# itsdevbear/go-avalanche

Measured on AMD Instinct MI355X. Metric: vote-record updates/sec (node·target·round) at 1/2/4/8 GPU; % HBM roofline, higher is better.
Workload: dtype u32; 1 GPU; C4: 1M nodes x 1000 targets, k=8, Bernoulli(0.8) initial acceptance, honest, sim mode; n_nodes=1000000, n_targets=1000, k=8, parallelism=single GPU

## Files before the change

go-avalanche_amd/csrc/engine.cpp:

```cpp
#include <algorithm>
#include <cstdarg>
#include <cstdio>
#include <cstring>
#include <memory>
#include <string>
#include <utility>
#include <vector>

#include "engine.h"

using namespace aveng;

namespace aveng {

static thread_local std::string g_last_error;

int fail(int code, const char* fmt, ...) {
  char buf[512];
  va_list ap;
  va_start(ap, fmt);
  vsnprintf(buf, sizeof(buf), fmt, ap);
  va_end(ap);
  g_last_error = buf;
  return code;
// ... 41 lines not shown
  p.log_shards = e->log_shards;
  p.n_nodes = (uint32_t)e->N;
  p.n0 = (uint32_t)e->n0;
  p.NL = e->NL;
  p.BL = e->BL;
  p.PS = e->PS;
  p.L = e->L;
  p.Lpad = e->Lpad;
  p.t0 = (uint32_t)e->t0;
  p.round = (uint32_t)e->round;
  p.round_rel = (uint32_t)(e->round - e->log_base);
  p.round_shift = e->round_shift;
  p.peer_mode = e->cfg.peer_mode;
  p.warm_all = e->facts.warm_all ? 1u : 0u;
  p.store_policy = e->store_policy;
  p.bl_magic = e->bl_magic;
  p.bl_sh1 = e->bl_sh1;
  p.bl_sh2 = e->bl_sh2;
  p.kpend = e->kpend;
  p.tn = (uint32_t)(e->t1 - e->t0);
  p.nopipe = e->sweep_nopipe ? 1u : 0u;
  p.tpw = e->wave_runs && e->sweep_blocks ? 1u : 0u;
  p.settled_fast = e->settled_fast ? 1u : 0u;
  p.lean = e->settled_lean && 64 % e->BL == 0 ? 1u : 0u;
  p.bl_log2 = (uint32_t)__builtin_ctz(e->BL);
  p.pub_mode = (uint32_t)e->pub_mode;
  p.readd = e->pub_mode == 2 ? e->readd : nullptr;
  p.died_out = e->pub_mode == 2 ? e->died_out : nullptr;
  p.nopoll = e->any_nopoll ? e->nopoll : nullptr;
  p.dense_min = e->dense_min;
  p.wave_dense = e->wave_dense;
  p.uni_votes = e->uni_votes;
  p.quiet_tiles = e->quiet_tiles;
  return p;
}

int materialize(av_engine* e, bool votes, bool counts) {
  votes = votes && e->facts.v_stale;
  counts = counts && e->facts.k_pend;
  if (!votes && !counts) return AV_OK;
  AV_HIP(avk::launch_materialize(round_params(e, nullptr), votes, counts, e->stream));
  if (votes) e->facts.votes_written_back();
  if (counts) e->facts.counts_written_back();
  return AV_OK;
}
int materialize_votes(av_engine* e) { return materialize(e, true, true); }

int engine_scratch(av_engine* e, size_t bytes, void** out) {
  const hipError_t he = e->fetch_scratch.reserve(bytes);
  AV_CHECK(he == hipSuccess, oom_or_hip(he), "scratch (%zu B): %s", bytes, hipGetErrorString(he));
  *out = e->fetch_scratch;
  return AV_OK;
}

int ref_pick(av_engine* e) {
  if (e->ref_node != -1) return AV_OK;
  e->ref_node = -2;
  const size_t words = std::min<size_t>((e->N + 31) / 32, 1024);
  std::vector<uint32_t> w(words);
  AV_HIP(hipMemcpyAsync(w.data(), e->byz, words * 4, hipMemcpyDeviceToHost, e->stream));
  AV_HIP(hipStreamSynchronize(e->stream));
  for (size_t i = 0; i < words && e->ref_node < 0; ++i)
    if (~w[i]) {
      const int64_t n = (int64_t)i * 32 + __builtin_ctz(~w[i]);
      if (n < e->N) e->ref_node = n;
    }
// ... 378 lines not shown
  e->log_shards = (uint32_t)std::max<uint64_t>(1, std::min<uint64_t>(waves, avk::kLogShards));
  e->log_cap = (uint32_t)std::max<int64_t>((cap + e->log_shards - 1) / e->log_shards, 64);
  AV_TRY(created(e->planes.alloc(plane_words), "alloc planes"));
  e->rflag_off = (pref_words * 4 + 255) / 256 * 256;
  e->uni_off = (e->rflag_off + (size_t)e->N + 255) / 256 * 256 / 4;
  e->pref_alloc_words =
      ((e->uni_off * 4 + (avk::kMaxPeers + 1) * 4 + (2u << 20) - 1) / (2u << 20)) * (2u << 20) / 4;
  for (auto& pref : e->pref) AV_TRY(created(pref.alloc_zeroed(e->pref_alloc_words, s), "alloc pref"));
  AV_TRY(created(e->vstale.alloc_zeroed(e->Lpad / 64, s), "alloc planes"));
  AV_TRY(created(e->kpend.alloc_zeroed(e->Lpad / 64, s), "alloc planes"));
  AV_TRY(created(e->valid.alloc(e->BL), "alloc valid"));
  AV_TRY(created(e->byz.alloc((e->N + 31) / 32), "alloc byz"));
  AV_TRY(created(e->log.alloc((size_t)e->log_cap * e->log_shards), "alloc log"));
  AV_TRY(created(e->log_count.alloc_zeroed(3 * avk::kLogShards * avk::kCtrStride, s), "alloc log"));
  e->mlog_count = e->log_count + avk::kLogShards * avk::kCtrStride;
  e->dlog_count = e->log_count + 2 * avk::kLogShards * avk::kCtrStride;
  const uint32_t dw = avk::dense_words((uint32_t)e->k);
  e->dense_min = avk::dense_min((uint32_t)e->k);
  const uint32_t dense_least = e->k == 8 ? 4u : e->dense_min;
  e->dlog_cap = std::max<uint32_t>(e->log_cap / dense_least, 16);
  AV_TRY(created(e->dlog.alloc((size_t)e->dlog_cap * e->log_shards * dw), "alloc log"));
  AV_TRY(created(e->upd_count.alloc_zeroed(avk::kLogShards, s), "alloc log"));
  e->mlog_cap = e->k == 8 ? std::max<uint32_t>(e->log_cap / 2, 16) : 16u;
  AV_TRY(created(e->mlog.alloc((size_t)e->mlog_cap * e->log_shards * avk::med_rec_words()), "alloc log"));
  e->log_alloc = (size_t)e->log_cap * e->log_shards;
  e->mlog_alloc = (size_t)e->mlog_cap * e->log_shards;
  e->dlog_alloc = (size_t)e->dlog_cap * e->log_shards;
  AV_TRY(created(e->log_overflow.alloc_zeroed(1, s), "alloc log"));
  if (e->capped) AV_TRY(created(e->node_flags.alloc_zeroed(e->NL, s), "alloc node flags"));
  AV_TRY(created(e->applied.alloc_zeroed(avk::kLogShards, s), "alloc counters"));
  AV_TRY(created(e->bytes.alloc_zeroed(2 * avk::kLogShards, s), "alloc counters"));
  AV_TRY(created(e->finalized.alloc_zeroed(avk::kLogShards, s), "alloc counters"));
  AV_TRY(created(e->scratch_count.alloc(1), "alloc counters"));
  AV_TRY(created(e->changed.alloc_zeroed(3 * avk::kLogShards, s), "alloc counters"));
  AV_TRY(created(e->nq.alloc_zeroed(4, s), "alloc counters"));
  e->valid_host.assign(e->BL, 0u);
  for (uint32_t b = 0; b < e->BL; ++b) {
    const int64_t tb = e->t0 + 32ll * b;
    const int64_t r = std::min<int64_t>(e->t1 - tb, 32);
    e->valid_host[b] = r >= 32 ? ~0u : ((1u << r) - 1u);
  }
  AV_TRY(created(hipMemcpyAsync(e->valid, e->valid_host.data(), e->BL * 4, hipMemcpyHostToDevice, s), "upload valid"));
  AV_TRY(created(avk::launch_byz(e->byz, (uint32_t)e->N, c.seed, c.byz_threshold, s), "byz kernel"));
  e->sweep_blocks = default_sweep_blocks(e);
  set_log_layout(e);
  AV_TRY(av_init_records(e, AV_INIT_NONE, 0));
  *out = guard.release();
  return AV_OK;
}

int av_init_records(av_engine* e, int32_t init_mode, uint32_t init_param) {
  AV_ENTER(e);
  AV_CHECK(init_mode >= AV_INIT_NONE && init_mode <= AV_INIT_PAIRS, AV_ERR_INVALID_ARG, "bad init_mode");
  if (e->facts.v_stale) AV_HIP(hipMemsetAsync(e->vstale, 0, (size_t)(e->Lpad / 64) * 4, e->stream));
  if (e->facts.k_pend) AV_HIP(hipMemsetAsync(e->kpend, 0, (size_t)(e->Lpad / 64) * 4, e->stream));
  e->facts.init(init_mode != AV_INIT_NONE);
  avk::InitParams p{};
  p.planes = e->planes;
  p.pref = e->pref[e->cur];
  p.byz = e->byz;
  p.seed = e->cfg.seed;
  p.n_nodes = (uint32_t)e->N;
  p.n0 = (uint32_t)e->n0;
  p.NL = e->NL;
  p.BL = e->BL;
  p.PS = e->PS;
  p.L = e->L;
// ... 149 lines not shown
  return {n, kd, lo, hi, nullptr, nullptr, m};
}

constexpr PlainOption kPlainOptions[] = {
    opt("plane_nt", &av_engine::plane_nt),
    opt("uniform_rows", &av_engine::uni_rows),
    opt("ref_rows", &av_engine::ref_rows),
    opt("virtual_votes", &av_engine::virtual_votes),
    opt("vv_min_bl", &av_engine::vv_min_bl, kReject, 1, (1ll << 31) - 1),
    opt("kernel", &av_engine::kernel, kReject, 1, 2),
    opt("store_policy", &av_engine::store_policy, kReject, 0, 3),
    opt("settled_fast", &av_engine::settled_fast),
    opt("settled_lean", &av_engine::settled_lean),
    opt("wave_runs", &av_engine::wave_runs),
    opt("sweep_nopipe", &av_engine::sweep_nopipe),
    opt("uni_merge", &av_engine::uni_merge, kReject, 1, 16),
    opt("uni_votes", &av_engine::uni_votes),
    opt("quiet_tiles", &av_engine::quiet_tiles),
    opt("net_quiet", &av_engine::net_quiet),
    opt("net_quiet_group", &av_engine::nq_group, kReject, 1, 16),
    opt("net_quiet_front", &av_engine::nq_front),
    opt("wave_dense", &av_engine::wave_dense, kReject, 0, 64),
    opt("tile_draw", &av_engine::tile_draw, kReject, 0, 1),
    opt("materialize_run", &av_engine::mat_run, kReject, 1, 64),
    opt("replay_fuse", &av_engine::replay_fuse, kReject, 0, 4096),
    opt("replay_fast", &av_engine::replay_fast),
    opt("dropin_fast", &av_engine::dropin_fast),
    opt("push_defer", &av_engine::push_defer),
    opt("push_store", &av_engine::push_store, kReject, 0, 2),
    opt("census_blocks", &av_engine::census_blocks, kReject, 0, 65536),
    opt("copy_blocks", &av_engine::copy_blocks, kReject, 0, 4096),
    opt("enc_buckets", &av_engine::enc_buckets, kReject, 1, 1ll << 30),
    opt("count_changed", &av_engine::count_changed),
    opt("round_marker", &av_engine::round_marker),
    opt("warm_pref", &av_engine::warm_pref),
    opt("unsynced_shard", &av_engine::unsynced_shard),
    opt("ablate_gather", &av_engine::ablate_gather),
    opt("ablate_phase", &av_engine::ablate_phase, kClamp, 0, 31),
    opt("ablate_emit", &av_engine::ablate_emit, kClamp, 0, 3),
    opt("ablate_node", &av_engine::ablate_node, kClamp, 0, 7),
};

int opt_range(const char* name, int64_t value, int64_t lo, int64_t hi) {
  AV_CHECK(value >= lo && value <= hi, AV_ERR_INVALID_ARG, "%s must be in [%lld, %lld]", name, (long long)lo,
           (long long)hi);
  return AV_OK;
}

int set_plain(av_engine* e, const PlainOption& o, int64_t value) {
  if (o.kind == kReject) AV_TRY(opt_range(o.name, value, o.lo, o.hi));
  value = o.kind == kBool ? value != 0 : std::max(o.lo, std::min(o.hi, value));
  if (o.b)
    e->*o.b = value != 0;
  else if (o.u)
    e->*o.u = (uint32_t)value;
  else
    e->*o.i = (int)value;
  return AV_OK;
}

int opt_sweep_blocks(av_engine* e, int64_t value) {
  AV_TRY(opt_range("sweep_blocks", value, -2, (1ll << 31) - 1));
  AV_ENTER(e);
  e->sweep_blocks = value < 0 ? default_sweep_blocks(e, value == -2) : (uint32_t)value;
  e->sweep_blocks_explicit = value >= 0;
  return relayout_log_if_empty(e);
// ... 148 lines not shown
```

go-avalanche_amd/csrc/engine.h:

```cpp
#pragma once

#include <hip/hip_runtime.h>
#include <rccl/rccl.h>

#include <algorithm>
#include <cstdint>
#include <cstdlib>
#include <thread>
#include <utility>
#include <vector>

#pragma GCC visibility push(default)
#include "../../include/avhip.h"
#pragma GCC visibility pop
#include "engine_mem.h"
#include "kernels.h"
#include "round_plan.h"

namespace aveng {
int fail(int code, const char* fmt, ...) __attribute__((format(printf, 2, 3)));
inline int oom_or_hip(hipError_t he) { return he == hipErrorOutOfMemory ? AV_ERR_OOM : AV_ERR_HIP; }
}

#define AV_HIP(call)                                                                                           \
// ... 120 lines not shown
  bool pref_uncached = false;
  bool peer_fine = true;
  size_t pref_alloc_words = 0;
  uint32_t barrier_seq = 0;
  uint32_t barrier_timeout_ms = 30000;
  std::vector<void*> peer_opened;
  avk::PeerPtrs peer_arrive{};
  avmem::DevBuf<uint32_t*> push_tbl;
  uint64_t barrier_ticks = 0;
  bool solo_barrier = false;
  bool solo_used = false;
  PeerGroup* group = nullptr;
  bool peer_mask = true;
  bool push_defer = true;
  uint32_t push_store = 1;
  uint32_t tile_draw = 0;
  uint32_t mat_run = 1;
  uint32_t census_blocks = 0;
  bool masked = false;
  uint32_t segs = 1;
  avmem::DevBuf<uint8_t> need_mine;
  avmem::DevBuf<uint8_t> needmask;
  avmem::DevBuf<uint8_t> stale;
  uint32_t* needin = nullptr;
  avmem::DevBuf<uint32_t> needin_own;
  avk::PeerPtrs peer_needin{};
  int64_t need_ready = -1;
  int64_t need_pushed = -1;
  avmem::Stream need_stream;
  avmem::Event need_free, need_drawn;
  int64_t need_drawn_w = -1;
  avmem::DevBuf<unsigned long long> changed;
  bool count_changed = false;
  int64_t rflag_clear_round = 0;

  uint32_t dense_min = 0;
  uint32_t wave_dense = 0;
  uint32_t uni_votes = 1;
  uint32_t quiet_tiles = 1;
  uint32_t net_quiet = 1;
  uint32_t nq_group = 16;
  uint32_t nq_front = 1;
  avmem::DevBuf<uint32_t> nq;
  int32_t pub_mode = 0;
  avmem::DevBuf<uint32_t> readd;
  avmem::DevBuf<uint32_t> died_out;
  std::vector<uint32_t> nopoll_host;
  avmem::DevBuf<uint32_t> nopoll;
  bool any_nopoll = false;
  std::vector<int64_t> proc_round;
  avmem::DevBuf<void> fetch_scratch;
  avmem::DevBuf<unsigned long long> digest;
  avmem::PinnedBuf<void> dropin_host;
  avmem::PinnedBuf<void> stage[2];
  avmem::Event stage_ev[2];
  bool dropin_fast = true;
  avmem::DevBuf<uint32_t> enc_err;
  avmem::DevBuf<uint64_t> enc_tot;
  uint32_t enc_buckets = 1u << 26;
  uint32_t copy_blocks = 0;
  static constexpr int kSlots = 3;
  avmem::Stream copy_stream;
  avmem::DevBuf<uint8_t> cdev[kSlots];
  avmem::PinnedBuf<uint8_t> chost[kSlots];
  avmem::Event cev[kSlots];
  av_compact_header chdr[kSlots] = {};
// ... 70 lines not shown
```

go-avalanche_amd/csrc/engine_records.cpp:

```cpp
#include <cstring>

#include "engine.h"

using namespace aveng;

namespace {

int peer_local_write_check(const av_engine* e) {
  AV_CHECK(e->peer_world <= 1, AV_ERR_UNSUPPORTED,
           "record writes outside a round are not supported on a peer-push node-sharded engine");
  return AV_OK;
}

int sum_shards(av_engine* e, const unsigned long long* dev, int64_t* out) {
  std::vector<unsigned long long> c(avk::kLogShards);
  AV_HIP(hipMemcpyAsync(c.data(), dev, avk::kLogShards * 8, hipMemcpyDeviceToHost, e->stream));
  AV_HIP(hipStreamSynchronize(e->stream));
  unsigned long long t = 0;
  for (auto v : c) t += v;
  *out = (int64_t)t;
  return AV_OK;
}

}
// ... 409 lines not shown
  if (out->target_classes) {
    const int64_t counted = (int64_t)h[tn * 4 + 256];
    for (size_t t = 0; t < tn; ++t) {
      int64_t* row = out->target_classes + t * AV_CENSUS_CLASSES;
      row[AV_CENSUS_LIVE_REJECTED] = (int64_t)h[t * 3];
      row[AV_CENSUS_LIVE_ACCEPTED] = (int64_t)h[t * 3 + 1];
      row[AV_CENSUS_ABSENT_ACCEPTED] = (int64_t)h[t * 3 + 2];
      row[AV_CENSUS_ABSENT_REJECTED] = counted - row[0] - row[1] - row[3];
    }
  }
  if (out->target_count_sum)
    for (size_t t = 0; t < tn; ++t) out->target_count_sum[t] = (int64_t)h[tn * 3 + t];
  if (out->count_hist)
    for (size_t i = 0; i < 256; ++i) out->count_hist[i] = (int64_t)h[tn * 4 + i];
  return AV_OK;
}

int av_alg_bytes(av_engine* e, int64_t* out) {
  AV_TRY(counter_query(e, out));
  return sum_shards(e, e->bytes, out);
}

int av_alg_bytes_reread(av_engine* e, int64_t* out) {
  AV_TRY(counter_query(e, out));
  return sum_shards(e, e->bytes + avk::kLogShards, out);
}

int av_changed_words(av_engine* e, int64_t* words, int64_t* segments) {
  AV_TRY(counter_query(e, words));
  AV_TRY(sum_shards(e, e->changed, words));
  return segments ? sum_shards(e, e->changed + avk::kLogShards, segments) : AV_OK;
}

int av_net_quiet_rounds(av_engine* e, int64_t* out) {
  AV_TRY(counter_query(e, out));
  uint32_t v = 0;
  AV_HIP(hipMemcpyAsync(&v, e->nq + 2, 4, hipMemcpyDeviceToHost, e->stream));
  AV_HIP(hipStreamSynchronize(e->stream));
  *out = (int64_t)v;
  return AV_OK;
}

int av_read_pref(av_engine* e, int64_t n0, int64_t n1, int64_t t0, int64_t t1, uint8_t* out) {
  AV_ENTER(e);
  AV_PEER_SYNC_CHECK(e);
  AV_CHECK(out && n0 >= 0 && n0 <= n1 && n1 <= e->N && t0 >= e->t0 && t0 <= t1 && t1 <= e->t1,
           AV_ERR_INVALID_ARG, "bad range");
  const size_t rows = (size_t)(n1 - n0);
  std::vector<uint32_t> w(rows * e->BL);
  if (rows) AV_TRY(av_read_pref_words(e, n0, n1, w.data()));
  const int64_t W = t1 - t0;
  for (size_t r = 0; r < rows; ++r)
    for (int64_t t = t0; t < t1; ++t) {
      const int64_t tl = t - e->t0;
      out[r * W + (t - t0)] = (uint8_t)((w[r * e->BL + (tl >> 5)] >> (tl & 31)) & 1u);
    }
  return AV_OK;
}

int av_read_pref_words(av_engine* e, int64_t n0, int64_t n1, uint32_t* out) {
  AV_ENTER(e);
  AV_PEER_SYNC_CHECK(e);
  AV_CHECK(out && n0 >= 0 && n0 <= n1 && n1 <= e->N, AV_ERR_INVALID_ARG, "bad range");
  const size_t words = (size_t)(n1 - n0) * e->BL;
  if (!words) return AV_OK;
  AV_HIP(hipMemcpy2DAsync(out, (size_t)e->BL * 4, e->pref[e->cur] + (size_t)n0 * e->PS, (size_t)e->PS * 4,
// ... 26 lines not shown
```

go-avalanche_amd/csrc/kernels.h:

```cpp
#pragma once

#include <hip/hip_runtime.h>
#include <stdint.h>

namespace avk {

constexpr int kPlanes = 25;
constexpr int kPV = 0, kPC = 8, kPA = 16, kPK = 17;
constexpr uint32_t kLogShards = 1024;
constexpr uint32_t kCtrStride = 32;
constexpr uint32_t kMaxPoll = 4096;
constexpr int kMaxK = 16;
constexpr int kMaxPeers = 15;

__host__ __device__ constexpr size_t replay_groups(int k) { return (size_t)((k + 1) / 2); }
__host__ __device__ inline size_t replay_words(uint32_t Lpad, int k) { return replay_groups(k) * 4u * Lpad; }
__host__ __device__ inline size_t replay_idx(uint32_t g, int k, int j, int c) {
  return (((size_t)(g >> 6) * replay_groups(k) + (size_t)(j >> 1)) * 64u + (g & 63u)) * 4u + (size_t)((j & 1) * 2 + c);
}

__host__ __device__ constexpr uint32_t pref_stride(uint32_t BL) {
  return BL > 32u ? (BL + 31u) / 32u * 32u : (BL <= 1u ? 1u : 1u << (32 - __builtin_clz(BL - 1u)));
}

// ... 77 lines not shown
  uint32_t ps_shift;
  const uint8_t* rflag_in;
  uint8_t* rflag_out;
  uint32_t rflag_off;

  uint32_t* uni_out;
  const uint32_t* uni_in;
  const uint32_t* uni_prev;
  uint32_t uni_world, uni_rank, uni_off;
  uint32_t uni_merge;
  uint32_t uni_post;

  uint32_t fresh;
  uint32_t tn;
  uint32_t hivirt;
  uint32_t tpw;
  uint32_t settled_fast;
  uint32_t lean;
  uint32_t bl_log2;
  uint32_t nopipe;
  uint32_t pub_mode;
  uint32_t* readd;
  uint32_t* died_out;
  const uint32_t* nopoll;
  uint32_t dense_min;
  uint32_t uni_votes;
  uint32_t quiet_tiles;
  uint32_t* nq_out;
  const uint32_t* nq_in;
  uint32_t* nq_rounds;
  uint32_t nq_group;
  uint32_t nq_front;
  uint32_t wave_dense;
};
constexpr uint32_t kPendAllLive = 0x80000000u;
constexpr uint32_t kHiVirt = 0x40000000u;
__host__ __device__ inline uint32_t real_mask(uint32_t tn, uint32_t b) {
  const uint32_t rem = tn > b * 32u ? tn - b * 32u : 0u;
  return rem >= 32u ? ~0u : ((1u << rem) - 1u);
}
constexpr uint32_t kVStale = 1u, kVUniform = 2u, kVMask = 3u, kCAll = 4u;

inline void bl_divider(uint32_t d, uint32_t& magic, uint32_t& sh1, uint32_t& sh2) {
  uint32_t l = 0;
  while ((1ull << l) < d) ++l;
  magic = (uint32_t)((((1ull << l) - d) << 32) / d + 1);
  sh1 = l < 1 ? l : 1;
  sh2 = l > 1 ? l - 1 : 0;
}

__host__ __device__ constexpr uint32_t dense_words(uint32_t k) { return (k + 5u) / 2u; }
__host__ __device__ constexpr uint32_t dense_min(uint32_t k) { return dense_words(k); }

constexpr uint32_t kMedS4Died = 1u << 8;
__host__ __device__ constexpr uint32_t med_rec_words() { return 4u; }

__host__ __device__ inline uint64_t pack_update(uint32_t round_rel, uint32_t node, uint32_t slot,
                                                uint32_t target, uint32_t status, uint32_t round_shift) {
  return ((uint64_t)round_rel << round_shift) | ((uint64_t)node << 28) | ((uint64_t)slot << 24) |
         ((uint64_t)target << 2) | (uint64_t)status;
}

hipError_t launch_round(const RoundParams& p, int k, bool replay, bool capped, hipStream_t s);
hipError_t launch_replay_node(const RoundParams& p, int k, hipStream_t s);
enum class SweepMode : int;
hipError_t launch_round_sweep(const RoundParams& p, int k, SweepMode mode, uint32_t blocks, hipStream_t s,
// ... 145 lines not shown
```

go-avalanche_amd/csrc/round_sweep.hip:

```cpp
#include <hip/hip_runtime.h>

#include <algorithm>

#include "kernels.h"
#include "round_common.h"
#include "round_plan.h"
#include "round_slots.h"

#ifndef AVK_ABLATE_PHASE
#define AVK_ABLATE_PHASE 0
#endif
#ifndef AVK_PUB_PRELOAD
#define AVK_PUB_PRELOAD 0
#endif

namespace avk {
namespace {

constexpr bool kAblatePhase = AVK_ABLATE_PHASE != 0;

struct SweepAcc {
  uint32_t applied = 0, died = 0, lane_bytes = 0;
  uint32_t reread = 0;
  uint32_t emitted_bytes = 0, updates = 0;
// ... 223 lines not shown
        if (in.stale == kVStale && (uflags & kUniPrev)) {
          const uint32_t rp = at_byte(p.pref_prev, p.ref_node * rb + bo);
          in.v0 = u32x4{rp, rp, rp, rp};
          in.v1 = u32x4{rp, rp, rp, 0u};
        } else if (in.stale == kVStale) {
          uint32_t pp[K];
          pick_parked(p, wd->sdp, wd->badp, base, x.node, p.round - 1u, rb, pp);
#pragma unroll
          for (int i = 0; i < 4; ++i) in.v0[i] = nog ? pp[7 - i] * 0x9E3779B9u : at_byte(p.pref_prev, pp[7 - i] + bo);
#pragma unroll
          for (int i = 0; i < 3; ++i) in.v1[i] = nog ? pp[3 - i] * 0x9E3779B9u : at_byte(p.pref_prev, pp[3 - i] + bo);
          in.v1[3] = 0u;
        }
        pick_parked(p, wd->sdc, wd->badc, base, x.node, p.round, rb, rows);
        drawn = have_rows = true;
        if (nog) {
#pragma unroll
          for (int j = 0; j < K; ++j) in.w[j] = (rows[j] + bo) * 0x9E3779B9u;
          return;
        }
      } else if (in.stale == kVStale) {
        const PairDraw pd = pair_draw(p, p.round, nlA, nn, lane);
        {
          uint32_t pp[K];
          pick_peers(p, pd, 0u, p.round, x.node, x.nl, nlA, nn, lane, pp);
#pragma unroll
          for (int i = 0; i < 4; ++i) in.v0[i] = p.pref_prev[pp[7 - i] * p.PS + x.b];
#pragma unroll
          for (int i = 0; i < 3; ++i) in.v1[i] = p.pref_prev[pp[3 - i] * p.PS + x.b];
          in.v1[3] = 0u;
        }
        pick_peers(p, pd, 1u, p.round, x.node, x.nl, nlA, nn, lane, peers);
        drawn = true;
      }
    }
    if (uflags & kUniVotes) {
      const uint32_t rw = at_byte(p.pref_prev, p.ref_node * rb + bo);
#pragma unroll
      for (int j = 0; j < K; ++j) in.w[j] = rw;
      return;
    }
    if (!drawn) draw_peers<K>(p, p.round, x.node, x.nl, nlA, nn, lane, peers);
    if (!have_rows) {
#pragma unroll
      for (int j = 0; j < K; ++j) rows[j] = (ABLATE ? x.node : peers[j]) * rb;
    }
#pragma unroll
    for (int j = 0; j < K; ++j) in.w[j] = at_byte(p.pref_in, rows[j] + bo);
  }
}

__device__ __forceinline__ uint8_t ref_tag(uint32_t snapshot_round) { return (uint8_t)(0x80u | (snapshot_round & 0x7Fu)); }

__device__ __forceinline__ void ref_flag_store(const RoundParams& p, uint32_t lane, bool active, uint32_t b,
                                               uint32_t node, uint32_t pub, uint32_t ref) {
  const uint64_t eq = __ballot(!active || pub == ref);
  const uint32_t s0 = lane - b;
  const uint64_t seg = (p.BL >= 64u ? ~0ull : ((1ull << p.BL) - 1ull)) << (s0 & 63u);
  if (active && b == 0u) {
    const uint8_t f = (eq & seg) == seg ? ref_tag(p.round + 1u) : 0u;
    if (p.push_n && p.rflag_out[node] != f) {
      for (uint32_t r = 0; r < p.push_n; ++r)
        __hip_atomic_store(reinterpret_cast<uint8_t*>(peer_ptr(p.push_dst, r)) + p.rflag_off + node, f, __ATOMIC_RELAXED,
                           __HIP_MEMORY_SCOPE_SYSTEM);
    }
    p.rflag_out[node] = f;
// ... 667 lines not shown
              const PairDraw dc = single_draw(p, p.round, nlA, nn, lane);
              wd.ok = !dp.fallback && !dc.fallback;
              if (wd.ok) {
                park_draw(dp, sd, lane, p.PS * 4u);
                park_draw(dc, sd + 256, lane, p.PS * 4u);
              }
              wd.sdp = sd;
              wd.sdc = sd + 256;
              wd.badp = dp.bad;
              wd.badc = dc.bad;
            } else {
              const PairDraw d = any_stale ? pair_draw(p, p.round, nlA, nn, lane) : single_draw(p, p.round, nlA, nn, lane);
              wd.ok = !d.fallback;
              if (wd.ok) park_draw(d, sd, lane, p.PS * 4u);
              wd.sdp = sd;
              wd.sdc = any_stale ? sd + 128 : sd;
              wd.badp = d.bad & 0xFFFFFFFFull;
              wd.badc = any_stale ? d.bad >> 32 : d.bad;
              wd.fofs = any_stale ? 32u : 0u;
              if constexpr (REF) {
                if (wd.ok && p.rflag_in && p.klazy) {
                  const uint8_t tag = ref_tag(p.round);
                  uint32_t ok = 1u;
#pragma unroll
                  for (int i = 0; i < 4; ++i) ok &= p.rflag_in[d.prod[i]] == tag ? 1u : 0u;
                  wd.flagok = __ballot(ok != 0u);
                }
              }
            }
          }
        }
      }
    }
    uint32_t lean_done = uni_done;
    bool lean_ran = uni_ran;
    if constexpr (MODE == kModeWarm && K == 8) {
      if (!uni_ran && wd.ok && wd.badc == 0ull && p.lean && p.settled_fast && p.klazy && p.vv && tile < tile_end) {
        lean_done = settled_run<POL, REF, CC>(p, lane, tile_end, wd, acc);
        lean_ran = true;
      }
    }
    const uint32_t qfirst = tile, qstep = stride;
    uint32_t qn = 0;
    if constexpr (MODE == kModeWarm && K == 8) {
      if (lean_ran && stride == 1u && tile < tile_end &&
          lean_done == (uint32_t)((1ull << (tile_end - tile)) - 1ull)) {
        qn = tile_end - tile;
        tile = tile_end;
      }
    }
    const bool tdraw = MODE == kModeWarm && K == 8 && p.tile_draw && p.tpw && !wd.ok && tile < tile_end;
    for (; tile < tile_end; tile += stride) {
      constexpr bool AB = MODE == kModeAblate;
      if constexpr (CC) acc.qslot = qn++;
      if constexpr (MODE == kModeWarm) {
        if constexpr (K == 8) {
          if (lean_done && ((lean_done >> (tile - wd.t0)) & 1u)) continue;
          if (tdraw) {
            const uint32_t tnlA = uni(div_bl(p, tile * 64u));
            const uint32_t tnn = uni(div_bl(p, min(tile * 64u + 64u, p.L) - 1u)) - tnlA + 1u;
            const bool tst = ((meta_of(wd, tile) >> 8) & kVMask) == kVStale;
            const PairDraw d = tst ? pair_draw(p, p.round, tnlA, tnn, lane) : single_draw(p, p.round, tnlA, tnn, lane);
            wd.ok = !d.fallback;
            if (wd.ok) {
              park_draw(d, sd, lane, p.PS * 4u);
              wd.nlA = tnlA;
              wd.nn = tnn;
              wd.pair = tst;
              wd.sdp = sd;
              wd.sdc = tst ? sd + 128 : sd;
              wd.badp = d.bad & 0xFFFFFFFFull;
              wd.badc = tst ? d.bad >> 32 : d.bad;
              wd.fofs = tst ? 32u : 0u;
              wd.flagok = 0ull;
            }
          }
          if (wd.ok && p.settled_fast && p.klazy && p.vv && !lean_ran) {
            const uint32_t m = meta_of(wd, tile);
            if (((m >> 8) & kVMask) == kVUniform && (m & kPendAllLive) &&
                settled_tile<POL, REF, CC>(p, tile, lane, m & (kPendAllLive | kHiVirt | 0xFFu), wd, acc))
              continue;
          }
        }
        TileIn<K, false, true> in;
        load_tile<K, false, true, POL, false, true, false, CC>(p, tile, lane, in, &wd, uflags);
        process_tile<K, false, true, POL, true, REF, CC>(p, tile, lane, in, 0u, acc, uflags);
      } else if constexpr (MODE == kModeFresh) {
        TileIn<K, false, false> in;
        load_tile<K, false, false, POL, false, true, true>(p, tile, lane, in);
        process_tile<K, false, false, POL, true>(p, tile, lane, in, 0u, acc);
      } else if constexpr (MODE == kModeReplay) {
        TileIn<K, true, false> in;
        load_tile<K, true, false, POL, false>(p, tile, lane, in);
        process_tile<K, true, false, POL>(p, tile, lane, in, 0u, acc);
      } else {
        bool warm = false;
        if (p.warm_skip) {
          const uint32_t g = tile * 64u + lane;
          const uint32_t c7 = g < p.L ? p.planes[(size_t)tile * (kPlanes * 64u) + 1024u + 7u * 64u + lane] : ~0u;
          warm = __all(c7 == ~0u);
        }
        if (warm) {
          TileIn<K, false, true> in;
          load_tile<K, false, true, POL, AB>(p, tile, lane, in);
          process_tile<K, false, true, POL>(p, tile, lane, in, 4u, acc);
        } else {
          TileIn<K, false, false> in;
          load_tile<K, false, false, POL, AB>(p, tile, lane, in);
          process_tile<K, false, false, POL>(p, tile, lane, in, 0u, acc);
        }
      }
    }
    if constexpr (CC) {
      if (p.push_q && qn) acc.pushed += (uint32_t)wave_sum(flush_pushes(p, lane, qfirst, qstep, qn, acc.qpub, acc.qpm));
    }
  }
  const unsigned long long s = wave_sum(acc.applied);
  const unsigned long long f = __ballot(acc.died != 0u) ? wave_sum(acc.died) : 0ull;
  const unsigned long long by = (unsigned long long)wave_sum(acc.lane_bytes) + acc.emitted_bytes;
  const unsigned long long rr = wave_sum(acc.reread);
  if (lane == 0) {
    const uint32_t shard = acc.shard;
// ... 43 lines not shown
        else
          hipLaunchKernelGGL((k_round_sweep<K, MODE, 3, false, CC>), dim3(grid), dim3(256), shm, s, p);
      }
  }
  return hipGetLastError();
}

template <int K, int MODE>
hipError_t launch_mode(const RoundParams& p, uint32_t grid, hipStream_t s) {
  if constexpr (K == 8 && MODE == kModeWarm) {
    if (!p.count_changed) return launch_mode_cc<K, MODE, false>(p, grid, s);
  }
  return launch_mode_cc<K, MODE, true>(p, grid, s);
}

template <int K>
hipError_t launch_sweep_k(const RoundParams& p_in, SweepMode mode, uint32_t blocks, hipStream_t s, bool* ref_written) {
  if (ref_written) *ref_written = false;
  const uint32_t tiles = p_in.Lpad / 64u;
  const SweepGrid g = sweep_grid(tiles, blocks);
  RoundParams p = p_in;
  p.tpw = 0u;
  p.push_q = p.push_defer && p.push_n && p.push_n <= 8u && g.run <= kPushQ ? 1u : 0u;
  if (mode == SweepMode::Warm && p_in.tpw && K == 8 && g.run && g.run <= 16u) {
    p.tpw = g.run;
    if (ref_written) *ref_written = p.rflag_out != nullptr;
    return launch_mode<K, kModeWarm>(p, g.grid, s);
  }
  p.rflag_out = nullptr;
  p.rflag_in = nullptr;
  switch (mode) {
    case SweepMode::Replay: return launch_mode<K, kModeReplay>(p, g.grid, s);
    case SweepMode::Ablate: return launch_mode<K, kModeAblate>(p, g.grid, s);
    case SweepMode::Fresh: return launch_mode<K, kModeFresh>(p, g.grid, s);
    case SweepMode::Warm:
      if (blocks && g.grid < (tiles + 3u) / 4u && !p.nopipe) {
        p.push_q = 0u;
        return launch_mode<K, kModeWarmPipe>(p, g.grid, s);
      }
      return launch_mode<K, kModeWarm>(p, g.grid, s);
    case SweepMode::Check: break;
  }
  return launch_mode<K, kModeCheck>(p, g.grid, s);
}

__device__ __forceinline__ void materialize_tile(const RoundParams& p, uint32_t tile, uint32_t lane, uint32_t raw,
                                                 uint32_t kw) {
  const LaneIdx x = lane_idx(p, tile, lane);
  uint32_t* const tp = p.planes + (size_t)tile * (kPlanes * 64u);
  u32x4* const grp = reinterpret_cast<u32x4*>(tp) + lane;
  const uint32_t st = raw & kVMask;
  const uint32_t pend = kw & 0xFFu;
  const bool dok = (pend || (kw & kHiVirt)) && x.active;
  u32x4 o0, o1, k0, k1;
  if (st == kVUniform) {
    const uint32_t A = tp[1536u + lane];
    o0 = o1 = u32x4{A, A, A, A};
  } else if (st) {
    const uint32_t nlA = uni(x.nl), nn = (uint32_t)__builtin_amdgcn_readlane((int)x.nl, 63) - nlA + 1u;
    uint32_t pp[8];
    draw_peers<8>(p, p.round - 1u, x.node, x.nl, nlA, nn, lane, pp);
#pragma unroll
    for (int c = 0; c < 4; ++c) {
      o0[c] = p.pref_prev[pp[7 - c] * p.PS + x.b];
      o1[c] = p.pref_prev[pp[3 - c] * p.PS + x.b];
    }
  }
  uint32_t vb = 0u;
  if (dok) {
    k0 = grp[128];
    k1 = kw & kHiVirt ? u32x4{0u, 0u, 0u, ~real_mask(p.tn, x.b)} : grp[192];
    vb = p.valid[x.b];
  }
  if ((raw & kCAll) && x.active) {
#pragma unroll
    for (int c = 0; c < 8; ++c) pst<true>(tp + 1024u + (uint32_t)c * 64u + lane, ~0u);
  }
  if (st && x.active) {
    pst4<true>(grp, o0);
    pst4<true>(grp + 64, o1);
  }
  if (dok) {
    uint32_t Kp[8];
#pragma unroll
    for (int c = 0; c < 4; ++c) {
      Kp[c] = k0[c];
      Kp[4 + c] = k1[c];
    }
    const uint32_t P0 = ~Kp[7] & vb;
    uint32_t cy = 0u;
#pragma unroll
    for (int c = 0; c < 4; ++c) {
      const uint32_t bi = ((pend >> c) & 1u) ? P0 : 0u;
      const uint32_t t = Kp[3 + c] ^ bi;
      const uint32_t si = t ^ cy;
      cy = (t & cy) | (Kp[3 + c] & bi);
      Kp[3 + c] = si;
    }
    u32x4 o2, o3;
#pragma unroll
    for (int c = 0; c < 4; ++c) {
      o2[c] = Kp[c];
      o3[c] = Kp[4 + c];
    }
    pst4<true>(grp + 128, o2);
    pst4<true>(grp + 192, o3);
  }
}

__global__ __launch_bounds__(256) void k_materialize(const RoundParams p, uint32_t run, uint32_t do_v, uint32_t do_k) {
  const uint32_t lane = threadIdx.x & 63u;
  const uint32_t wave = uni(blockIdx.x * 4u + (threadIdx.x >> 6));
  const uint32_t tiles = p.Lpad >> 6;
  if (run == 1u) {
    if (wave >= tiles) return;
    const uint32_t raw = do_v ? uni(p.vstale[wave]) : 0u;
    const uint32_t kw = do_k ? uni(p.kpend[wave]) : 0u;
    if (raw == 0u && kw == 0u) return;
    materialize_tile(p, wave, lane, raw, kw);
    if (lane == 0) {
      if (raw) p.vstale[wave] = 0u;
      if (kw) p.kpend[wave] = 0u;
    }
    return;
  }
  const uint32_t t0 = wave * run;
  if (t0 >= tiles) return;
  const uint32_t n = min(run, tiles - t0);
  const uint32_t ti = t0 + lane;
  const uint32_t stw = do_v && lane < n ? p.vstale[ti] : 0u;
  const uint32_t kww = do_k && lane < n ? p.kpend[ti] : 0u;
  if (__ballot(stw != 0u || kww != 0u) == 0ull) return;
  for (uint32_t i = 0; i < n; ++i) {
    const uint32_t raw = (uint32_t)__builtin_amdgcn_readlane((int)stw, (int)i);
    const uint32_t kw = (uint32_t)__builtin_amdgcn_readlane((int)kww, (int)i);
    if (raw == 0u && kw == 0u) continue;
    materialize_tile(p, t0 + i, lane, raw, kw);
  }
  if (lane < n) {
    if (stw) p.vstale[ti] = 0u;
    if (kww) p.kpend[ti] = 0u;
  }
}

template <int K>
hipError_t occupancy_k(bool replay, int* bpc) {
  return replay ? hipOccupancyMaxActiveBlocksPerMultiprocessor(bpc, k_round_sweep<K, kModeReplay, 1>, 256, 0)
                : hipOccupancyMaxActiveBlocksPerMultiprocessor(bpc, k_round_sweep<K, kModeWarmPipe, 1>, 256, 0);
}

}

#define AVK_SWEEP_SWITCH(k, CALL) \
  switch (k) {                    \
    case 1: return CALL(1);       \
    case 2: return CALL(2);       \
    case 3: return CALL(3);       \
    case 4: return CALL(4);       \
    case 5: return CALL(5);       \
    case 6: return CALL(6);       \
    case 7: return CALL(7);       \
    case 8: return CALL(8);       \
    default: return hipErrorInvalidValue; \
  }

hipError_t launch_round_sweep(const RoundParams& p, int k, SweepMode mode, uint32_t blocks, hipStream_t s,
                              bool* ref_written) {
#define AVK_SW(K) launch_sweep_k<K>(p, mode, blocks, s, ref_written)
  AVK_SWEEP_SWITCH(k, AVK_SW)
#undef AVK_SW
}

hipError_t launch_materialize(const RoundParams& p, bool do_v, bool do_k, hipStream_t s) {
  if ((do_v && (!p.vstale || !p.pref_prev)) || (do_k && !p.kpend)) return hipErrorInvalidValue;
  if (!do_v && !do_k) return hipSuccess;
// ... 20 lines not shown
```

go-avalanche_amd/python/avhip/__init__.py:

```python
from __future__ import annotations

import ctypes as C
import os

import numpy as np

try:
    import torch
except Exception:
    torch = None

_PKG_ROOT = os.path.dirname(os.path.dirname(os.path.dirname(os.path.abspath(__file__))))
LIB_PATH = os.environ.get("AVHIP_LIB") or os.path.join(_PKG_ROOT, "lib", "libavhip.so")
HEADER_PATH = os.path.join(os.path.dirname(_PKG_ROOT), "include", "avhip.h")

AV_OK = 0
AV_ERR_INVALID_ARG = -1
AV_ERR_NOT_FOUND = -4
AV_ERR_OVERFLOW = -5
AV_ERR_PEER = -8

STATUS_INVALID, STATUS_REJECTED, STATUS_ACCEPTED, STATUS_FINALIZED = 0, 1, 2, 3
PEERS_RANDOM, PEERS_ROUND_ROBIN = 0, 1
INIT_NONE, INIT_REJECTED, INIT_ACCEPTED, INIT_BERNOULLI, INIT_PAIRS = 0, 1, 2, 3, 4
# ... 31 lines not shown
        ("device", C.c_int32),
        ("node_begin", C.c_int64),
        ("node_end", C.c_int64),
        ("target_begin", C.c_int64),
        ("target_end", C.c_int64),
        ("update_log_capacity", C.c_int64),
    ]


class CensusOut(C.Structure):
    _fields_ = [
        ("target_classes", C.c_void_p),
        ("target_count_sum", C.c_void_p),
        ("node_classes", C.c_void_p),
        ("count_hist", C.c_void_p),
    ]


CENSUS_LIVE_REJECTED, CENSUS_LIVE_ACCEPTED, CENSUS_ABSENT_REJECTED, CENSUS_ABSENT_ACCEPTED = 0, 1, 2, 3

PEER_HANDLE_BYTES = 320

EXPORTED = [
    "av_abi_version", "av_config_init", "av_create", "av_destroy", "av_strerror", "av_last_error",
    "av_init_records", "av_add_targets", "av_set_valid", "av_register_votes", "av_is_accepted",
    "av_get_confidence", "av_get_invs", "av_get_invs_batch", "av_run_rounds", "av_replay_round_errs", "av_replay_prepare",
    "av_replay_rounds", "av_synchronize", "av_round_index", "av_updates_count", "av_fetch_updates",
    "av_update_log_overflowed", "av_applied_votes", "av_alg_bytes", "av_alg_bytes_reread", "av_finalized_count", "av_live_records", "av_census", "av_discard_updates", "av_read_records", "av_write_records", "av_read_pref", "av_sample_peers",
    "av_set_option", "av_set_timing", "av_kernel_stats", "av_layout_info", "av_comm_unique_id", "av_comm_init",
    "av_peer_handles", "av_peer_init", "av_get_round", "av_set_round", "av_log_base_round", "av_updates_digest",
    "av_updates_digest_range", "av_read_pref_words", "av_set_polling",
    "av_register_votes_batch", "av_changed_words", "av_materialize", "av_peer_group_serial", "av_peer_sync",
    "av_pushed_words", "av_log_entries", "av_resize_log", "av_fetch_compact", "av_fetch_compact_async",
    "av_fetch_compact_wait", "av_compact_expand", "av_update_round_shift", "av_net_quiet_rounds",
]

_lib = None
_vp = C.c_void_p


def lib():
    global _lib
    if _lib is not None:
        return _lib
    if not os.path.exists(LIB_PATH):
        raise OSError(f"libavhip.so not built at {LIB_PATH} (run __graft_entry__.build() or make -C go-avalanche_amd)")
    L = C.CDLL(LIB_PATH)
    i64, i32, u32 = C.c_int64, C.c_int32, C.c_uint32
    P = C.POINTER
    sig = {
        "av_abi_version": (i32, []),
        "av_config_init": (None, [P(Config)]),
        "av_create": (i32, [P(Config), P(_vp)]),
        "av_destroy": (i32, [_vp]),
        "av_strerror": (C.c_char_p, [i32]),
        "av_last_error": (C.c_char_p, []),
        "av_init_records": (i32, [_vp, i32, u32]),
        "av_add_targets": (i32, [_vp, i64, _vp, _vp, i64, _vp]),
        "av_set_valid": (i32, [_vp, i64, i32]),
        "av_register_votes": (i32, [_vp, i64, _vp, _vp, i64, _vp]),
        "av_is_accepted": (i32, [_vp, i64, i64, P(i32)]),
        "av_get_confidence": (i32, [_vp, i64, i64, P(C.c_uint16)]),
        "av_get_invs": (i32, [_vp, i64, _vp, i64, P(i64)]),
        "av_get_invs_batch": (i32, [_vp, i64, i64, _vp, _vp, i64, P(i64)]),
        "av_run_rounds": (i32, [_vp, i32]),
        "av_replay_round_errs": (i32, [_vp, _vp]),
        "av_replay_prepare": (i32, [_vp, i32]),
        "av_replay_rounds": (i32, [_vp, i32]),
        "av_synchronize": (i32, [_vp]),
        "av_round_index": (i32, [_vp, P(i64)]),
        "av_updates_count": (i32, [_vp, P(i64)]),
        "av_fetch_updates": (i32, [_vp, _vp, i64, P(i64)]),
        "av_update_log_overflowed": (i32, [_vp, P(i32)]),
        "av_applied_votes": (i32, [_vp, P(i64)]),
        "av_alg_bytes": (i32, [_vp, P(i64)]),
        "av_alg_bytes_reread": (i32, [_vp, P(i64)]),
        "av_net_quiet_rounds": (i32, [_vp, P(i64)]),
        "av_changed_words": (i32, [_vp, P(i64), P(i64)]),
        "av_materialize": (i32, [_vp]),
        "av_finalized_count": (i32, [_vp, P(i64)]),
        "av_live_records": (i32, [_vp, i32, P(i64)]),
        "av_census": (i32, [_vp, i64, i64, i32, P(CensusOut)]),
        "av_discard_updates": (i32, [_vp]),
        "av_read_records": (i32, [_vp, i64, i64, i64, i64, _vp]),
        "av_write_records": (i32, [_vp, i64, i64, i64, i64, _vp]),
        "av_read_pref": (i32, [_vp, i64, i64, i64, i64, _vp]),
        "av_sample_peers": (i32, [_vp, i64, i64, i64, _vp]),
        "av_set_option": (i32, [_vp, C.c_char_p, i64]),
        "av_set_timing": (i32, [_vp, i32]),
        "av_kernel_stats": (i32, [_vp, P(C.c_double), P(i64)]),
        "av_layout_info": (i32, [_vp, P(i64), P(i64), P(i64), P(i32)]),
        "av_comm_unique_id": (i32, [_vp]),
        "av_comm_init": (i32, [_vp, i32, i32, _vp]),
        "av_peer_handles": (i32, [_vp, _vp]),
        "av_peer_init": (i32, [_vp, i32, i32, _vp]),
        "av_get_round": (i32, [_vp, i64, P(i64)]),
        "av_set_round": (i32, [_vp, i64, i64]),
        "av_log_base_round": (i32, [_vp, P(i64)]),
        "av_updates_digest": (i32, [_vp, _vp]),
        "av_updates_digest_range": (i32, [_vp, i64, i64, _vp]),
        "av_read_pref_words": (i32, [_vp, i64, i64, _vp]),
        "av_set_polling": (i32, [_vp, i64, i32]),
        "av_register_votes_batch": (i32, [_vp, i64, _vp, _vp, _vp, _vp, _vp]),
        "av_peer_group_serial": (i32, [_vp, i32]),
        "av_peer_sync": (i32, [_vp]),
        "av_pushed_words": (i32, [_vp, P(i64)]),
        "av_log_entries": (i32, [_vp, _vp]),
        "av_resize_log": (i32, [_vp, _vp]),
        "av_fetch_compact": (i32, [_vp, _vp, i64, P(i64)]),
        "av_fetch_compact_async": (i32, [_vp, P(i64)]),
        "av_fetch_compact_wait": (i32, [_vp, i64, P(_vp), P(i64)]),
        "av_compact_expand": (i32, [_vp, i64, _vp, i64, P(i64)]),
        "av_update_round_shift": (i32, [_vp, P(i32)]),
    }
    for name, (res, args) in sig.items():
        if name == "av_net_quiet_rounds" and os.environ.get("AVHIP_LIB") and not hasattr(L, name):
            continue
        f = getattr(L, name)
        f.restype = res
        f.argtypes = args
    _lib = L
    return L


def _check(rc):
    if rc == AV_OK:
        return
    msg = lib().av_last_error().decode(errors="replace")
    if rc == AV_ERR_NOT_FOUND:
        raise VoteRecordNotFound(rc, msg)
    if rc == AV_ERR_OVERFLOW:
        raise LogOverflow(rc, msg)
    if rc == AV_ERR_PEER:
        raise PeerExchangeFailed(rc, msg)
    raise AvError(rc, msg)


def _ptr(a: np.ndarray):
    return a.ctypes.data_as(_vp)


def decode_updates(u: np.ndarray, base_round: int = 0, round_shift: int = 52) -> np.ndarray:
    u = np.asarray(u, np.uint64)
    out = np.empty((u.size, 5), np.int64)
    out[:, 0] = (u >> np.uint64(round_shift)).astype(np.int64) + base_round
    out[:, 1] = ((u >> np.uint64(28)) & np.uint64((1 << (round_shift - 28)) - 1)).astype(np.int64)
    out[:, 2] = ((u >> np.uint64(24)) & np.uint64(0xF)).astype(np.int64)
    out[:, 3] = ((u >> np.uint64(2)) & np.uint64(0x3FFFFF)).astype(np.int64)
    out[:, 4] = (u & np.uint64(3)).astype(np.int64)
# ... 294 lines not shown
        if nodes:
            res["node_classes"] = np.zeros((max(0, n1 - n0), 4), np.int32)
        if hist:
            res["count_hist"] = np.zeros((2, 128), np.int64)
        out = CensusOut(*[res[k].ctypes.data if k in res else None
                          for k in ("target_classes", "target_count_sum", "node_classes", "count_hist")])
        _check(lib().av_census(self._h, n0, n1, int(honest_only), C.byref(out)))
        return res

    def log_overflowed(self) -> bool:
        v = C.c_int32()
        _check(lib().av_update_log_overflowed(self._h, C.byref(v)))
        return bool(v.value)

    def discard_updates(self):
        _check(lib().av_discard_updates(self._h))

    def alg_bytes(self):
        out = C.c_int64(0)
        _check(lib().av_alg_bytes(self._h, C.byref(out)))
        return out.value

    def alg_bytes_reread(self):
        out = C.c_int64(0)
        _check(lib().av_alg_bytes_reread(self._h, C.byref(out)))
        return out.value

    @property
    def net_quiet_rounds(self):
        out = C.c_int64(0)
        _check(lib().av_net_quiet_rounds(self._h, C.byref(out)))
        return out.value

    def changed_words(self):
        w, g = C.c_int64(0), C.c_int64(0)
        _check(lib().av_changed_words(self._h, C.byref(w), C.byref(g)))
        return w.value, g.value

    def log_entries(self):
        out = np.zeros(3, np.int64)
        _check(lib().av_log_entries(self._h, _ptr(out)))
        return tuple(int(v) for v in out)

    def resize_log(self, singles, slots, dense):
        v = np.array([singles, slots, dense], np.int64)
        _check(lib().av_resize_log(self._h, _ptr(v)))

    def pushed_words(self):
        out = C.c_int64(0)
        _check(lib().av_pushed_words(self._h, C.byref(out)))
        return out.value

    def peer_sync(self):
        _check(lib().av_peer_sync(self._h))

    def materialize(self):
        _check(lib().av_materialize(self._h))

    def read_records(self, n0=None, n1=None, t0=None, t1=None):
        n0 = self.node_range[0] if n0 is None else n0
        n1 = self.node_range[1] if n1 is None else n1
        t0 = self.target_range[0] if t0 is None else t0
        t1 = self.target_range[1] if t1 is None else t1
        out = np.zeros((n1 - n0, t1 - t0), np.uint32)
        _check(lib().av_read_records(self._h, n0, n1, t0, t1, _ptr(out)))
        return out
# ... 52 lines not shown
```

include/avhip.h:

```cpp
#ifndef AVHIP_H
#define AVHIP_H

#include <stdint.h>

#ifdef __cplusplus
extern "C" {
#endif

#define AVHIP_ABI_VERSION 1

#define AV_OK 0
#define AV_ERR_INVALID_ARG (-1)
#define AV_ERR_HIP (-2)
#define AV_ERR_OOM (-3)
#define AV_ERR_NOT_FOUND (-4)
#define AV_ERR_OVERFLOW (-5)
#define AV_ERR_UNSUPPORTED (-6)
#define AV_ERR_RCCL (-7)
#define AV_ERR_PEER (-8)

#define AV_STATUS_INVALID 0
#define AV_STATUS_REJECTED 1
#define AV_STATUS_ACCEPTED 2
#define AV_STATUS_FINALIZED 3
// ... 94 lines not shown
  int32_t target_bits;
  int32_t slot_bits;
  int32_t round_shift;
  int32_t reserved;
} av_compact_header;
int av_fetch_compact(av_engine* e, void* out, int64_t cap, int64_t* bytes);
int av_fetch_compact_async(av_engine* e, int64_t* ticket);
int av_fetch_compact_wait(av_engine* e, int64_t ticket, const void** stream, int64_t* bytes);
int av_compact_expand(const void* stream, int64_t bytes, uint64_t* out, int64_t cap, int64_t* n_out);
int av_updates_digest(av_engine* e, uint64_t out[3]);
int av_updates_digest_range(av_engine* e, int64_t n0, int64_t n1, uint64_t out[3]);
int av_applied_votes(av_engine* e, int64_t* out);
int av_finalized_count(av_engine* e, int64_t* out);
int av_live_records(av_engine* e, int32_t honest_only, int64_t* out);
#define AV_CENSUS_LIVE_REJECTED   0
#define AV_CENSUS_LIVE_ACCEPTED   1
#define AV_CENSUS_ABSENT_REJECTED 2
#define AV_CENSUS_ABSENT_ACCEPTED 3
#define AV_CENSUS_CLASSES 4
typedef struct {
  int64_t* target_classes;
  int64_t* target_count_sum;
  int32_t* node_classes;
  int64_t* count_hist;
} av_census_out;
int av_census(av_engine* e, int64_t n0, int64_t n1, int32_t honest_only, const av_census_out* out);
int av_discard_updates(av_engine* e);
int av_log_entries(av_engine* e, int64_t out[3]);
int av_resize_log(av_engine* e, const int64_t entries[3]);
int av_alg_bytes(av_engine* e, int64_t* out);
int av_alg_bytes_reread(av_engine* e, int64_t* out);
int av_net_quiet_rounds(av_engine* e, int64_t* out);
int av_changed_words(av_engine* e, int64_t* words, int64_t* segments);
int av_materialize(av_engine* e);
int av_read_records(av_engine* e, int64_t n0, int64_t n1, int64_t t0, int64_t t1, uint32_t* out);
int av_write_records(av_engine* e, int64_t n0, int64_t n1, int64_t t0, int64_t t1, const uint32_t* in);
int av_read_pref(av_engine* e, int64_t n0, int64_t n1, int64_t t0, int64_t t1, uint8_t* out);
int av_read_pref_words(av_engine* e, int64_t n0, int64_t n1, uint32_t* out);
int av_sample_peers(av_engine* e, int64_t round, int64_t n0, int64_t n1, int32_t* out);

int av_set_option(av_engine* e, const char* name, int64_t value);

int av_set_timing(av_engine* e, int32_t enable);
int av_kernel_stats(av_engine* e, double* total_ms, int64_t* launches);
int av_layout_info(av_engine* e, int64_t* lanes, int64_t* local_nodes, int64_t* local_blocks, int32_t* capped);

int av_comm_unique_id(uint8_t out[128]);
int av_comm_init(av_engine* e, int32_t world, int32_t rank, const uint8_t id[128]);

#define AV_PEER_HANDLE_BYTES 320
int av_peer_handles(av_engine* e, uint8_t out[AV_PEER_HANDLE_BYTES]);
int av_peer_init(av_engine* e, int32_t world, int32_t rank, const uint8_t* handles);
int av_peer_group_serial(av_engine** engines, int32_t world);
int av_peer_sync(av_engine* e);
int av_pushed_words(av_engine* e, int64_t* out);

#ifdef __cplusplus
}
#endif
#endif
```

Before: 30900 billion vote-record updates/s (1 update = 1 regsiterVote on a live record; k=8 per node·target·round).

## Draw peers once per multi-tile wave run in fresh sweep; lean count writeback

In fresh mode with k=8, each wave now handles a run of consecutive tiles and draws a single peer sample for the whole node range, parking it and reusing it in load_tile. The aim is to cut per-tile peer-draw work. Materialize also skips reading and writing the low count plane when no low pending bit is set (wb_lean), which trims writeback traffic. An optional writeback byte counter with its API is added; it is off by default and costs extra atomics when enabled.

```diff
diff --git a/go-avalanche_amd/csrc/engine.cpp b/go-avalanche_amd/csrc/engine.cpp
--- a/go-avalanche_amd/csrc/engine.cpp
+++ b/go-avalanche_amd/csrc/engine.cpp
@@ -97,6 +97,9 @@
   p.wave_dense = e->wave_dense;
   p.uni_votes = e->uni_votes;
   p.quiet_tiles = e->quiet_tiles;
+  p.wb_lean = e->wb_lean;
+  p.wb_bytes = e->wb_count ? e->changed + 3 * avk::kLogShards : nullptr;
+  p.fresh_runs = e->fresh_runs ? 1u : 0u;
   return p;
 }
 
@@ -541,7 +544,7 @@
   AV_TRY(created(e->bytes.alloc_zeroed(2 * avk::kLogShards, s), "alloc counters"));
   AV_TRY(created(e->finalized.alloc_zeroed(avk::kLogShards, s), "alloc counters"));
   AV_TRY(created(e->scratch_count.alloc(1), "alloc counters"));
-  AV_TRY(created(e->changed.alloc_zeroed(3 * avk::kLogShards, s), "alloc counters"));
+  AV_TRY(created(e->changed.alloc_zeroed(4 * avk::kLogShards, s), "alloc counters"));
   AV_TRY(created(e->nq.alloc_zeroed(4, s), "alloc counters"));
   e->valid_host.assign(e->BL, 0u);
   for (uint32_t b = 0; b < e->BL; ++b) {
@@ -757,6 +760,9 @@
     opt("copy_blocks", &av_engine::copy_blocks, kReject, 0, 4096),
     opt("enc_buckets", &av_engine::enc_buckets, kReject, 1, 1ll << 30),
     opt("count_changed", &av_engine::count_changed),
+    opt("wb_count", &av_engine::wb_count),
+    opt("wb_lean", &av_engine::wb_lean),
+    opt("fresh_runs", &av_engine::fresh_runs),
     opt("round_marker", &av_engine::round_marker),
     opt("warm_pref", &av_engine::warm_pref),
     opt("unsynced_shard", &av_engine::unsynced_shard),
diff --git a/go-avalanche_amd/csrc/engine.h b/go-avalanche_amd/csrc/engine.h
--- a/go-avalanche_amd/csrc/engine.h
+++ b/go-avalanche_amd/csrc/engine.h
@@ -176,6 +176,9 @@
   int64_t need_drawn_w = -1;
   avmem::DevBuf<unsigned long long> changed;
   bool count_changed = false;
+  bool wb_count = false;
+  uint32_t wb_lean = 1;
+  bool fresh_runs = true;
   int64_t rflag_clear_round = 0;
 
   uint32_t dense_min = 0;
diff --git a/go-avalanche_amd/csrc/engine_records.cpp b/go-avalanche_amd/csrc/engine_records.cpp
--- a/go-avalanche_amd/csrc/engine_records.cpp
+++ b/go-avalanche_amd/csrc/engine_records.cpp
@@ -465,6 +465,11 @@
   return segments ? sum_shards(e, e->changed + avk::kLogShards, segments) : AV_OK;
 }
 
+int av_writeback_bytes(av_engine* e, int64_t* out) {
+  AV_TRY(counter_query(e, out));
+  return sum_shards(e, e->changed + 3 * avk::kLogShards, out);
+}
+
 int av_net_quiet_rounds(av_engine* e, int64_t* out) {
   AV_TRY(counter_query(e, out));
   uint32_t v = 0;
diff --git a/go-avalanche_amd/csrc/kernels.h b/go-avalanche_amd/csrc/kernels.h
--- a/go-avalanche_amd/csrc/kernels.h
+++ b/go-avalanche_amd/csrc/kernels.h
@@ -133,6 +133,9 @@
   uint32_t nq_group;
   uint32_t nq_front;
   uint32_t wave_dense;
+  uint32_t wb_lean;
+  unsigned long long* wb_bytes;
+  uint32_t fresh_runs;
 };
 constexpr uint32_t kPendAllLive = 0x80000000u;
 constexpr uint32_t kHiVirt = 0x40000000u;
diff --git a/go-avalanche_amd/csrc/round_sweep.hip b/go-avalanche_amd/csrc/round_sweep.hip
--- a/go-avalanche_amd/csrc/round_sweep.hip
+++ b/go-avalanche_amd/csrc/round_sweep.hip
@@ -279,6 +279,12 @@
         }
         pick_peers(p, pd, 1u, p.round, x.node, x.nl, nlA, nn, lane, peers);
         drawn = true;
+      }
+    }
+    if constexpr (FRESH && K == 8) {
+      if (wd && wd->ok) {
+        pick_parked(p, wd->sdc, wd->badc, (x.nl - wd->nlA) * 2u, x.node, p.round, rb, rows);
+        drawn = have_rows = true;
       }
     }
     if (uflags & kUniVotes) {
@@ -1012,6 +1018,26 @@
         }
       }
     }
+    if constexpr (MODE == kModeFresh && K == 8) {
+      if (p.tpw) {
+        tile = wave0 * p.tpw;
+        tile_end = min(tile + p.tpw, tiles);
+        stride = 1u;
+        nq_tag = tile < tiles;
+        if (tile < tiles) {
+          const uint32_t nlA = uni(div_bl(p, tile * 64u));
+          const uint32_t nlB = uni(div_bl(p, min(tile_end * 64u, p.L) - 1u));
+          const PairDraw d = single_draw(p, p.round, nlA, nlB - nlA + 1u, lane);
+          wd.ok = !d.fallback;
+          if (wd.ok) park_draw(d, sd, lane, p.PS * 4u);
+          wd.sdc = sd;
+          wd.badc = d.bad;
+          wd.t0 = tile;
+          wd.nlA = nlA;
+          wd.nn = nlB - nlA + 1u;
+        }
+      }
+    }
     uint32_t lean_done = uni_done;
     bool lean_ran = uni_ran;
     if constexpr (MODE == kModeWarm && K == 8) {
@@ -1067,7 +1093,7 @@
         process_tile<K, false, true, POL, true, REF, CC>(p, tile, lane, in, 0u, acc, uflags);
       } else if constexpr (MODE == kModeFresh) {
         TileIn<K, false, false> in;
-        load_tile<K, false, false, POL, false, true, true>(p, tile, lane, in);
+        load_tile<K, false, false, POL, false, true, true>(p, tile, lane, in, &wd);
         process_tile<K, false, false, POL, true>(p, tile, lane, in, 0u, acc);
       } else if constexpr (MODE == kModeReplay) {
         TileIn<K, true, false> in;
@@ -1177,7 +1203,9 @@
   switch (mode) {
     case SweepMode::Replay: return launch_mode<K, kModeReplay>(p, g.grid, s);
     case SweepMode::Ablate: return launch_mode<K, kModeAblate>(p, g.grid, s);
-    case SweepMode::Fresh: return launch_mode<K, kModeFresh>(p, g.grid, s);
+    case SweepMode::Fresh:
+      if (p_in.fresh_runs && p_in.tpw && K == 8 && g.run && g.run <= 16u) p.tpw = g.run;
+      return launch_mode<K, kModeFresh>(p, g.grid, s);
     case SweepMode::Warm:
       if (blocks && g.grid < (tiles + 3u) / 4u && !p.nopipe) {
         p.push_q = 0u;
@@ -1189,15 +1217,16 @@
   return launch_mode<K, kModeCheck>(p, g.grid, s);
 }
 
-__device__ __forceinline__ void materialize_tile(const RoundParams& p, uint32_t tile, uint32_t lane, uint32_t raw,
-                                                 uint32_t kw) {
+__device__ __forceinline__ uint32_t materialize_tile(const RoundParams& p, uint32_t tile, uint32_t lane, uint32_t raw,
+                                                     uint32_t kw) {
   const LaneIdx x = lane_idx(p, tile, lane);
   uint32_t* const tp = p.planes + (size_t)tile * (kPlanes * 64u);
   u32x4* const grp = reinterpret_cast<u32x4*>(tp) + lane;
   const uint32_t st = raw & kVMask;
   const uint32_t pend = kw & 0xFFu;
   const bool dok = (pend || (kw & kHiVirt)) && x.active;
-  u32x4 o0, o1, k0, k1;
+  const bool klo = (pend & 1u) || !p.wb_lean;
+  u32x4 o0, o1, k0 = u32x4{0u, 0u, 0u, 0u}, k1;
   if (st == kVUniform) {
     const uint32_t A = tp[1536u + lane];
     o0 = o1 = u32x4{A, A, A, A};
@@ -1213,7 +1242,7 @@
   }
   uint32_t vb = 0u;
   if (dok) {
-    k0 = grp[128];
+    if (klo) k0 = grp[128];
     k1 = kw & kHiVirt ? u32x4{0u, 0u, 0u, ~real_mask(p.tn, x.b)} : grp[192];
     vb = p.valid[x.b];
   }
@@ -1248,9 +1277,13 @@
       o2[c] = Kp[c];
       o3[c] = Kp[4 + c];
     }
-    pst4<true>(grp + 128, o2);
+    if (klo) pst4<true>(grp + 128, o2);
     pst4<true>(grp + 192, o3);
   }
+  if (!p.wb_bytes) return 0u;
+  const uint32_t per_lane = (st == kVUniform ? 4u : st ? 32u : 0u) + (st ? 32u : 0u) + ((raw & kCAll) ? 32u : 0u) +
+                            (pend || (kw & kHiVirt) ? (klo ? 32u : 0u) + ((kw & kHiVirt) ? 16u : 32u) : 0u);
+  return per_lane * (uint32_t)__popcll(__ballot(x.active));
 }
 
 __global__ __launch_bounds__(256) void k_materialize(const RoundParams p, uint32_t run, uint32_t do_v, uint32_t do_k) {
@@ -1262,10 +1295,11 @@
     const uint32_t raw = do_v ? uni(p.vstale[wave]) : 0u;
     const uint32_t kw = do_k ? uni(p.kpend[wave]) : 0u;
     if (raw == 0u && kw == 0u) return;
-    materialize_tile(p, wave, lane, raw, kw);
+    const uint32_t moved = materialize_tile(p, wave, lane, raw, kw);
     if (lane == 0) {
       if (raw) p.vstale[wave] = 0u;
       if (kw) p.kpend[wave] = 0u;
+      if (p.wb_bytes && moved) atomicAdd(&p.wb_bytes[wave % kLogShards], (unsigned long long)moved);
     }
     return;
   }
@@ -1276,16 +1310,18 @@
   const uint32_t stw = do_v && lane < n ? p.vstale[ti] : 0u;
   const uint32_t kww = do_k && lane < n ? p.kpend[ti] : 0u;
   if (__ballot(stw != 0u || kww != 0u) == 0ull) return;
+  uint32_t moved = 0u;
   for (uint32_t i = 0; i < n; ++i) {
     const uint32_t raw = (uint32_t)__builtin_amdgcn_readlane((int)stw, (int)i);
     const uint32_t kw = (uint32_t)__builtin_amdgcn_readlane((int)kww, (int)i);
     if (raw == 0u && kw == 0u) continue;
-    materialize_tile(p, t0 + i, lane, raw, kw);
+    moved += materialize_tile(p, t0 + i, lane, raw, kw);
   }
   if (lane < n) {
     if (stw) p.vstale[ti] = 0u;
     if (kww) p.kpend[ti] = 0u;
   }
+  if (lane == 0 && p.wb_bytes && moved) atomicAdd(&p.wb_bytes[wave % kLogShards], (unsigned long long)moved);
 }
 
 template <int K>
diff --git a/go-avalanche_amd/python/avhip/__init__.py b/go-avalanche_amd/python/avhip/__init__.py
--- a/go-avalanche_amd/python/avhip/__init__.py
+++ b/go-avalanche_amd/python/avhip/__init__.py
@@ -87,7 +87,7 @@
     "av_updates_digest_range", "av_read_pref_words", "av_set_polling",
     "av_register_votes_batch", "av_changed_words", "av_materialize", "av_peer_group_serial", "av_peer_sync",
     "av_pushed_words", "av_log_entries", "av_resize_log", "av_fetch_compact", "av_fetch_compact_async",
-    "av_fetch_compact_wait", "av_compact_expand", "av_update_round_shift", "av_net_quiet_rounds",
+    "av_fetch_compact_wait", "av_compact_expand", "av_update_round_shift", "av_net_quiet_rounds", "av_writeback_bytes",
 ]
 
 _lib = None
@@ -131,6 +131,7 @@
         "av_alg_bytes": (i32, [_vp, P(i64)]),
         "av_alg_bytes_reread": (i32, [_vp, P(i64)]),
         "av_net_quiet_rounds": (i32, [_vp, P(i64)]),
+        "av_writeback_bytes": (i32, [_vp, P(i64)]),
         "av_changed_words": (i32, [_vp, P(i64), P(i64)]),
         "av_materialize": (i32, [_vp]),
         "av_finalized_count": (i32, [_vp, P(i64)]),
@@ -169,7 +170,7 @@
         "av_update_round_shift": (i32, [_vp, P(i32)]),
     }
     for name, (res, args) in sig.items():
-        if name == "av_net_quiet_rounds" and os.environ.get("AVHIP_LIB") and not hasattr(L, name):
+        if name in ("av_net_quiet_rounds", "av_writeback_bytes") and os.environ.get("AVHIP_LIB") and not hasattr(L, name):
             continue
         f = getattr(L, name)
         f.restype = res
@@ -530,6 +531,11 @@
         _check(lib().av_net_quiet_rounds(self._h, C.byref(out)))
         return out.value
 
+    def writeback_bytes(self):
+        out = C.c_int64(0)
+        _check(lib().av_writeback_bytes(self._h, C.byref(out)))
+        return out.value
+
     def changed_words(self):
         w, g = C.c_int64(0), C.c_int64(0)
         _check(lib().av_changed_words(self._h, C.byref(w), C.byref(g)))
diff --git a/include/avhip.h b/include/avhip.h
--- a/include/avhip.h
+++ b/include/avhip.h
@@ -150,6 +150,7 @@
 int av_alg_bytes_reread(av_engine* e, int64_t* out);
 int av_net_quiet_rounds(av_engine* e, int64_t* out);
 int av_changed_words(av_engine* e, int64_t* words, int64_t* segments);
+int av_writeback_bytes(av_engine* e, int64_t* out);
 int av_materialize(av_engine* e);
 int av_read_records(av_engine* e, int64_t n0, int64_t n1, int64_t t0, int64_t t1, uint32_t* out);
 int av_write_records(av_engine* e, int64_t n0, int64_t n1, int64_t t0, int64_t t1, const uint32_t* in);
```

New measurement: 31930 billion vote-record updates/s (1 update = 1 regsiterVote on a live record; k=8 per node·target·round), median of 6. 3.3% higher.
